# NCAR/SPERR

Hardware: AMD Instinct MI355X
Metric: compress+decompress GB/s/GPU on 256^3 fp32 chunks @ BPP=2.0; bitstream-exact vs ref (higher is better)
Workload: dtype f64; 1 GPU; synthetic 1024^3 fp32 turbulence per GPU, 256^3 chunks, BPP=2.0, step = compress + decompress, volume and container resident in HBM; chunks_per_gpu=64, parallelism=chunks farmed over 1 GPU(s), no collective

## Files before the change

### sperr_amd/csrc/xform.hip

```cpp
#include <type_traits>

#include "xform.h"
#include "speck_dec.h"

namespace sperrhip {


constexpr int kSumStrides = 64, kSumSeg = 64;


template <typename T>
__global__ void __launch_bounds__(kThreads)
k_stride_sums(const T* __restrict__ vol, VolDesc vd, const ChunkGeom* geom, uint32_t cx,
              uint32_t cy, uint32_t cz, uint32_t nstrides, uint32_t ssz, double* strideMean,
              size_t strideMeanStride, CoderState* st, int want_range)
{
  __shared__ double tile[kSumStrides][kSumSeg + 1];
  __shared__ uint32_t sh_differs;
  double vmax = -INFINITY, vnegmax = -INFINITY;
  const uint32_t c = blockIdx.y;
  const uint32_t s0 = blockIdx.x * kSumStrides;
  const ChunkGeom g = geom[c];
  const size_t vx = vd.dims[0], vy = vd.dims[1];
  const T first = vol[((size_t)g.org[2] * vy + g.org[1]) * vx + g.org[0]];
  if (threadIdx.x == 0)
    sh_differs = 0;
  double acc = 0.0;
  bool differs = false;
  (void)cz;
  for (uint32_t seg = 0; seg < ssz; seg += kSumSeg) {
    const uint32_t len = min((uint32_t)kSumSeg, ssz - seg);
    __syncthreads();
    for (uint32_t k = threadIdx.x; k < (uint32_t)(kSumStrides * kSumSeg); k += kThreads) {
      const uint32_t r = k / kSumSeg, j = k % kSumSeg;
      const uint32_t sidx = s0 + r;
      if (sidx < nstrides && j < len) {
        const uint32_t e = sidx * ssz + seg + j;
        const uint32_t x = e % cx, q = e / cx;
        const uint32_t y = q % cy, z = q / cy;
        const T v = vol[((size_t)(g.org[2] + z) * vy + (g.org[1] + y)) * vx + g.org[0] + x];
        differs |= (v != first);
        tile[r][j] = (double)v;
        vmax = fmax(vmax, (double)v);
        vnegmax = fmax(vnegmax, -(double)v);
      }
    }
    __syncthreads();
    if (threadIdx.x < (uint32_t)kSumStrides && s0 + threadIdx.x < nstrides)
      for (uint32_t j = 0; j < len; j++)
        acc += tile[threadIdx.x][j];
  }
  if (differs)
    sh_differs = 1;
  __syncthreads();
  if (threadIdx.x < (uint32_t)kSumStrides && s0 + threadIdx.x < nstrides)
    strideMean[c * strideMeanStride + s0 + threadIdx.x] = acc / (double)ssz;
  if (threadIdx.x == 0 && sh_differs)
    st[c].not_const_flag = 1;
  if (want_range) {
    for (int d = 32; d > 0; d >>= 1) {
      vmax = fmax(vmax, __shfl_xor(vmax, d, 64));
      vnegmax = fmax(vnegmax, __shfl_xor(vnegmax, d, 64));
    }
    if ((threadIdx.x & 63) == 0) {
      atomicMax(reinterpret_cast<unsigned long long*>(&st[c].vmaxKey), order_key(vmax));
      atomicMax(reinterpret_cast<unsigned long long*>(&st[c].vnegmaxKey), order_key(vnegmax));
    }
  }
}

template <typename T>
__global__ void __launch_bounds__(64)
k_stride_sums_rows(const T* __restrict__ vol, VolDesc vd, const ChunkGeom* geom, uint32_t cx,
                   uint32_t cy, uint32_t nstrides, uint32_t ssz, double* strideMean,
                   size_t strideMeanStride, CoderState* st, int want_range)
{
  constexpr int V = 16 / sizeof(T);
  struct alignas(16) Pack { T v[V]; };
  const uint32_t c = blockIdx.y;
  const uint32_t sidx = blockIdx.x * 64 + threadIdx.x;
  const ChunkGeom g = geom[c];
  const size_t vx = vd.dims[0], vy = vd.dims[1];
  const T first = vol[((size_t)g.org[2] * vy + g.org[1]) * vx + g.org[0]];
  double acc = 0.0, vmax = -INFINITY, vnegmax = -INFINITY;
  bool differs = false;
// ... 304 lines not shown
          EV(i) = fma(EV(i), K.inv_eps, -t);
        }
      __syncthreads();
      odd_step(-K.gamma);
      even_step(-K.beta);
      odd_step(-K.alpha);
    }
#undef EV
#undef OD
  }

  auto crop_store = [&](uint32_t l, uint32_t p, VT v) {
    uint32_t xyz[3];
    xyz[axis] = p;
    xyz[ua] = u0 + l;
    xyz[wa] = tw;
    if (crop_has(cg, xyz[0], xyz[1], xyz[2]))
      vol[crop_addr(cg, vd, xyz[0], xyz[1], xyz[2])] = v;
  };
  (void)crop_store;
  const bool wantMax = FORWARD && F.mode == 1 && !is_const;
  double vmax = 0.0;
  if (axis == 0) {
    const uint32_t nseg = (len + 63) / 64;
    for (uint32_t sg = tid / 64; sg < nl * nseg; sg += kThreads / 64) {
      const uint32_t l = sg / nseg, p = (sg % nseg) * 64 + tid % 64;
      if (p >= len)
        continue;
      const uint32_t src = FORWARD ? p : ((p & 1) ? even_len + (p >> 1) : (p >> 1));
      if constexpr (kCrop)
        crop_store(l, p, (VT)(is_const ? mean : sm[src * NLP + l] + mean));
      else if (IO != 0 && !FORWARD)
        vol[vbase + l * vsu + p * vsl] = (VT)(is_const ? mean : sm[src * NLP + l] + mean);
      else {
        const double v = sm[src * NLP + l];
        tile[l * su + p] = v;
        size_t idx;
        if (wantMax && outside_inner(l, p, idx))
          vmax = fmax(vmax, fabs(v));
      }
    }
  }
  else {
    const uint32_t l = tid % NL, k0 = tid / NL, kg = kThreads / NL;
    if (l < nl)
      for (uint32_t p = k0; p < len; p += kg) {
        const uint32_t src = FORWARD ? p : ((p & 1) ? even_len + (p >> 1) : (p >> 1));
        if constexpr (kCrop)
          crop_store(l, p, (VT)(is_const ? mean : sm[src * NLP + l] + mean));
        else if (IO != 0 && !FORWARD)
          vol[vbase + l * vsu + p * vsl] = (VT)(is_const ? mean : sm[src * NLP + l] + mean);
        else {
          const double v = sm[src * NLP + l];
          tile[l * su + p * sl] = v;
          size_t idx;
          if (wantMax && outside_inner(l, p, idx))
            vmax = fmax(vmax, fabs(v));
        }
      }
  }
  if (FORWARD && F.mode == 1) {
    for (int d = 32; d > 0; d >>= 1)
      vmax = fmax(vmax, __shfl_xor(vmax, d, 64));
    if ((tid & 63) == 0 && vmax > 0.0)
      atomicMax(reinterpret_cast<unsigned long long*>(&st[c].maxabs),
                (unsigned long long)__double_as_longlong(vmax));
  }
}

constexpr int kXYHalo = 4;
constexpr int kXYThreads = 512;
constexpr int kStage = 16;
constexpr int kSeg = 8;

__device__ __forceinline__ uint32_t reflect_index(int q, int n)
{
  const int period = 2 * (n - 1);
  q = q < 0 ? -q : q;
  if (q >= period)
    q %= period;
  return (uint32_t)(q < n ? q : period - q);
}

template <bool FORWARD>
__device__ __forceinline__ void lift16(double (&r)[16], const LiftConsts& K)
{
  if (FORWARD) {
#pragma unroll
    for (int k = 1; k <= 13; k += 2)
      r[k] = fma(K.alpha, r[k - 1] + r[k + 1], r[k]);
#pragma unroll
    for (int k = 2; k <= 12; k += 2)
      r[k] = fma(K.beta, r[k - 1] + r[k + 1], r[k]);
#pragma unroll
    for (int k = 3; k <= 11; k += 2)
      r[k] = fma(K.gamma, r[k - 1] + r[k + 1], r[k]);
#pragma unroll
    for (int k = 4; k <= 10; k += 2)
      r[k] = K.eps * fma(K.delta, r[k - 1] + r[k + 1], r[k]);
#pragma unroll
    for (int k = 5; k <= 11; k += 2)
      r[k] = (-K.inv_eps) * r[k];
  }
  else {
#pragma unroll
    for (int k = 1; k <= 15; k += 2)
      r[k] = (-K.eps) * r[k];
#pragma unroll
    for (int k = 2; k <= 14; k += 2) {
      const double t = K.delta * (r[k - 1] + r[k + 1]);
      r[k] = fma(r[k], K.inv_eps, -t);
    }
#pragma unroll
    for (int k = 3; k <= 13; k += 2)
      r[k] = fma(-K.gamma, r[k - 1] + r[k + 1], r[k]);
#pragma unroll
    for (int k = 4; k <= 12; k += 2)
      r[k] = fma(-K.beta, r[k - 1] + r[k + 1], r[k]);
#pragma unroll
    for (int k = 5; k <= 11; k += 2)
      r[k] = fma(-K.alpha, r[k - 1] + r[k + 1], r[k]);
  }
}

template <bool FORWARD, int IO, bool kCrop = false>
__global__ void __launch_bounds__(kXYThreads)
k_lift_xy(double* vals, size_t valsStride, uint32_t cx, uint32_t cy, uint32_t cz, int R,
          LiftConsts K, const CoderState* st, void* volume, VolDesc vd, const GeomOf<kCrop>* geom)
{
  static_assert(IO == 1 || IO == 2, "float or double volume");
  static_assert(!kCrop || !FORWARD, "the crop variant is a last inverse pass");
  using VT = typename std::conditional<IO == 1, float, double>::type;
  const uint32_t c = blockIdx.y;
  const bool is_const = st[c].is_const != 0;
  if (is_const && FORWARD)
    return;
  double* sm = reinterpret_cast<double*>(dyn_smem);
  const uint32_t ntile = (cy + R - 1) / R;
  const uint32_t z = blockIdx.x / ntile, y0 = (blockIdx.x % ntile) * R;
  const uint32_t ylo = y0 >= (uint32_t)kXYHalo ? y0 - kXYHalo : 0u;
  const uint32_t yhi = min(cy, y0 + R + kXYHalo);
  const uint32_t yend = min(cy, y0 + R);
  const uint32_t nrow = yhi - ylo;
  const uint32_t RS = cx + 1;
  const uint32_t xe = cx - cx / 2, ye = cy - cy / 2;
  const GeomOf<kCrop> g = geom[c];
  VT* vol = reinterpret_cast<VT*>(volume);
  const size_t vsy = vd.dims[0], vsz = (size_t)vd.dims[0] * vd.dims[1];
  size_t vbase = 0;
  uint32_t wy0 = y0, wy1 = yend, wx0 = 0, wx1 = cx;
  if constexpr (kCrop) {
    wy0 = max(y0, g.lo[1]);
    wy1 = min(yend, g.hi[1]);
    wx0 = g.lo[0];
    wx1 = g.hi[0];
    if (z - g.lo[2] >= g.hi[2] - g.lo[2] || wy0 >= wy1)
      return;
  }
  else
    vbase = (size_t)(g.org[2] + z) * vsz + (size_t)g.org[1] * vsy + g.org[0];
  auto out_at = [&](uint32_t x, uint32_t y) -> size_t {
    if constexpr (kCrop)
      return crop_addr(g, vd, x, y, z);
    else
      return vbase + (size_t)y * vsy + x;
  };
  double* buf = vals + c * valsStride + (size_t)z * cx * cy;
  const double mean = st[c].mean;
  const uint32_t tid = threadIdx.x;

  if (is_const) {
    if constexpr (kCrop) {
      const uint32_t w = wx1 - wx0;
      for (uint32_t k = tid; k < (wy1 - wy0) * w; k += kXYThreads)
        vol[out_at(wx0 + k % w, wy0 + k / w)] = (VT)mean;
    }
    else
      for (uint32_t k = tid; k < (yend - y0) * cx; k += kXYThreads)
        vol[vbase + (size_t)(y0 + k / cx) * vsy + k % cx] = (VT)mean;
    return;
  }

  const uint32_t lane = tid & 63u, wave = tid >> 6, nwaves = kXYThreads / 64;
  {
    using ST = typename std::conditional<FORWARD, VT, double>::type;
    const uint32_t nxb = (cx + 63) / 64;
    const uint32_t rowsW = nrow > wave ? (nrow - wave + nwaves - 1) / nwaves : 0;
    const uint32_t items = rowsW * nxb;
    uint32_t ri = 0, bi = 0;
    for (uint32_t m0 = 0; m0 < items; m0 += kStage) {
      ST v[kStage];
      uint32_t ri2 = ri, bi2 = bi;
#pragma unroll
      for (int u = 0; u < kStage; u++) {
        const uint32_t j = wave + nwaves * ri2, x = lane + 64 * bi2;
        v[u] = 0;
        if (m0 + u < items && x < cx) {
          const uint32_t y = ylo + j;
          if (FORWARD)
            v[u] = (ST)vol[vbase + (size_t)y * vsy + x];
          else
            v[u] = (ST)buf[(size_t)((y & 1) ? ye + (y >> 1) : (y >> 1)) * cx + ((x & 1) ? xe + (x >> 1) : (x >> 1))];
        }
        if (++bi2 == nxb) {
          bi2 = 0;
          ri2++;
// ... 62 lines not shown
      for (int k = 0; k < 16; k++) {
        const uint32_t yy = min(max(reflect_index(s - 4 + k, (int)cy), ylo), yhi - 1);
        r[k] = col[(size_t)(yy - ylo) * RS];
      }
    }
  };

  if (FORWARD) {
    lift_x(0, nrow);
    for (uint32_t xb = 0; xb < cx; xb += cpr) {
      const uint32_t x = xb + tid % cpr, q = tid / cpr;
      if (x < cx && q < nq) {
        double r[16];
        load_column(x, q, r);
        lift16<true>(r, K);
        const uint32_t dcol = (x & 1) ? xe + (x >> 1) : (x >> 1);
#pragma unroll
        for (int k = 0; k < kSeg; k++) {
          const uint32_t y = y0 + q * kSeg + k;
          if (y < yend)
            buf[(size_t)((y & 1) ? ye + (y >> 1) : (y >> 1)) * cx + dcol] = r[4 + k];
        }
      }
    }
  }
  else {
    for (uint32_t xb = 0; xb < cx; xb += cpr) {
      const uint32_t x = xb + tid % cpr, q = tid / cpr;
      const bool on = x < cx && q < nq;
      double r[16];
      if (on) {
        load_column(x, q, r);
        lift16<false>(r, K);
      }
      __syncthreads();
      if (on) {
#pragma unroll
        for (int k = 0; k < kSeg; k++) {
          const uint32_t y = y0 + q * kSeg + k;
          if (y < yend)
            sm[(size_t)(y - ylo) * RS + x] = r[4 + k];
        }
      }
    }
    __syncthreads();
    lift_x(y0 - ylo, yend - ylo);
    if constexpr (kCrop) {
      for (uint32_t y = wy0 + wave; y < wy1; y += nwaves) {
        VT* dstrow = vol + out_at(wx0, y);
        const double* srow = sm + (size_t)(y - ylo) * RS;
        for (uint32_t x = wx0 + lane; x < wx1; x += 64)
          dstrow[x - wx0] = (VT)(srow[x] + mean);
      }
    }
    else
    for (uint32_t y = y0 + wave; y < yend; y += nwaves) {
      VT* dstrow = vol + vbase + (size_t)y * vsy;
      const double* srow = sm + (size_t)(y - ylo) * RS;
      for (uint32_t x = lane; x < cx; x += 64)
        dstrow[x] = (VT)(srow[x] + mean);
    }
  }
}

#ifndef XYZ_INV_THREADS
#define XYZ_INV_THREADS 1024
#endif
#ifndef XYZ_INV_PREFETCH
#define XYZ_INV_PREFETCH 2
#endif
#ifndef XYZ_FWD_THREADS
#define XYZ_FWD_THREADS 1024
#endif
constexpr int kXYZThreadsF = XYZ_FWD_THREADS, kXYZThreadsI = XYZ_INV_THREADS;
constexpr int kXYZRows = 16;
constexpr int kXYZStaged = kXYZRows + 2 * kXYHalo;
constexpr int kXYZPosF = (4096 + kXYZThreadsF - 1) / kXYZThreadsF;
constexpr int kXYZStageF = (6144 + kXYZThreadsF - 1) / kXYZThreadsF;
constexpr int kXYZPosI = 6144 / kXYZThreadsI;
#ifndef XYZ_INV_GROUP
#define XYZ_INV_GROUP 3
#endif
constexpr int kXYZGroupI = XYZ_INV_GROUP;
constexpr int kXYZBoxSlots = 48;

__host__ __device__ inline uint32_t xyz_row_stride(uint32_t cx)
{
  return ((cx + 7u) & ~7u) + 9u;
}

#define XYZ_LDS_BARRIER() asm volatile("s_waitcnt lgkmcnt(0)\n\ts_barrier" ::: "memory")

__device__ __forceinline__ void xyz_put(double* row, uint32_t x, uint32_t cx, double v)
{
  row[4 + x] = v;
  if (x - 1u < 4u)
    row[4 - x] = v;
  if (cx - 2u - x < 4u)
    row[2 * cx + 2 - x] = v;
}

template <bool FORWARD, int NT>
__device__ __forceinline__ void xyz_lift_x(const double* src, double* dst, uint32_t RS, uint32_t cx, uint32_t jlo,
                                           uint32_t jhi, uint32_t tid, const LiftConsts& K)
{
  const uint32_t nseg = (cx + kSeg - 1) / kSeg;
  const uint32_t ntask = (jhi - jlo) * nseg;
#pragma unroll 1
  for (uint32_t t = tid; t < ntask; t += NT) {
    const uint32_t rows = jhi - jlo, sg = t / rows, rb = jlo + (t - sg * rows);
    const double* row = src + (size_t)rb * RS + sg * kSeg;
    double r[16];
#pragma unroll
    for (int k = 0; k < 16; k++)
      r[k] = row[k];
    lift16<FORWARD>(r, K);
    double* out = dst + (size_t)rb * RS + 4 + sg * kSeg;
#pragma unroll
    for (int k = 0; k < kSeg; k++)
      if (sg * kSeg + k < cx)
        out[k] = r[4 + k];
  }
}

template <bool FORWARD, bool APRON, int NT>
__device__ __forceinline__ void xyz_lift_y(const double* src, double* dst, uint32_t RS, uint32_t cx, uint32_t nt,
                                           uint32_t tid, const LiftConsts& K)
{
  const uint32_t nq = (nt + kSeg - 1) / kSeg;
  const uint32_t ntask = nq * cx;
#pragma unroll 1
  for (uint32_t t = tid; t < ntask; t += NT) {
    const uint32_t q = t / cx, x = t - q * cx;
    const double* top = src + (size_t)(q * kSeg) * RS + 4 + x;
    double r[16];
#pragma unroll
    for (int k = 0; k < 16; k++)
      r[k] = top[(size_t)k * RS];
    lift16<FORWARD>(r, K);
#pragma unroll
    for (int k = 0; k < kSeg; k++) {
      if (q * kSeg + k < nt) {
        double* row = dst + (size_t)(4 + q * kSeg + k) * RS;
        if (APRON)
          xyz_put(row, x, cx, r[4 + k]);
        else
          row[4 + x] = r[4 + k];
      }
    }
  }
}

template <int IO>
__global__ void __launch_bounds__(kXYZThreadsF) __attribute__((amdgpu_waves_per_eu(kXYZThreadsF / 256, kXYZThreadsF / 256)))
k_lift_xyz_fwd(double* vals, size_t valsStride, uint32_t cx, uint32_t cy, uint32_t cz, LiftConsts K,
               CoderState* st, const void* volume, VolDesc vd, const ChunkGeom* geom, int wantMax,
               uint32_t in0, uint32_t in1, uint32_t in2, uint32_t nseg)
{
  static_assert(IO == 1 || IO == 2, "float or double volume");
  using VT = typename std::conditional<IO == 1, float, double>::type;
  const uint32_t c = blockIdx.y;
  if (st[c].is_const != 0)
    return;
  const uint32_t tid = threadIdx.x;
  const uint32_t seg = blockIdx.x % nseg, npairsAll = (cz + 1) / 2;
  const uint32_t mA = seg == 0 ? 0u : (uint32_t)((uint64_t)npairsAll * seg / nseg);
  const uint32_t mB = seg + 1 == nseg ? npairsAll : (uint32_t)((uint64_t)npairsAll * (seg + 1) / nseg);
  const uint32_t zFirst = mA >= 6 ? 2 * (mA - 6) : 0u;
  const uint32_t zEnd = seg + 1 == nseg ? cz : 2 * mB - 1;
  const uint32_t y0 = (blockIdx.x / nseg) * kXYZRows;
  const uint32_t nt = min((uint32_t)kXYZRows, cy - y0);
  const uint32_t RS = xyz_row_stride(cx);
  double* sm = reinterpret_cast<double*>(dyn_smem);
  const uint32_t bufN = (uint32_t)kXYZStaged * RS;
  const uint32_t xe = cx - cx / 2, ye = cy - cy / 2, ze = cz - cz / 2;
  const VT* vol = reinterpret_cast<const VT*>(volume);
  const size_t vsy = vd.dims[0], vsz = (size_t)vd.dims[0] * vd.dims[1];
  const VT* volc = vol + ((size_t)geom[c].org[2] * vsz + (size_t)geom[c].org[1] * vsy + geom[c].org[0]);
  double* buf = vals + c * valsStride;
  const size_t sliceN = (size_t)cx * cy;
  const double mean = st[c].mean;

  const uint32_t nstage = (uint32_t)kXYZStaged * cx;
  uint32_t pk[kXYZStageF];
#pragma unroll
  for (int k = 0; k < kXYZStageF; k++) {
    const uint32_t q = tid + (uint32_t)k * kXYZThreadsF;
    const uint32_t j = q / cx, x = q - j * cx;
    pk[k] = (j << 27) | (reflect_index((int)y0 - kXYHalo + (int)j, (int)cy) << 12) | x;
  }
  const uint32_t npos = nt * cx;
  uint32_t srow[kXYZPosF], ooff[kXYZPosF];
  uint32_t outerMask = 0;
#pragma unroll
  for (int k = 0; k < kXYZPosF; k++) {
    const uint32_t q = tid + (uint32_t)k * kXYZThreadsF;
    const uint32_t row = q / cx, col = q - row * cx, y = y0 + row;
    srow[k] = ((row + kXYHalo) << 16) | col;
    const uint32_t drow = (y & 1) ? ye + (y >> 1) : (y >> 1), dcol = (col & 1) ? xe + (col >> 1) : (col >> 1);
    ooff[k] = drow * cx + dcol;
    if (!(dcol < in0 && drow < in1))
      outerMask |= 1u << k;
  }
  double sxe[kXYZPosF], sxo[kXYZPosF], d1p[kXYZPosF], e1p[kXYZPosF], d2p[kXYZPosF];
#pragma unroll
  for (int k = 0; k < kXYZPosF; k++)
    sxe[k] = sxo[k] = d1p[k] = e1p[k] = d2p[k] = 0.0;
  double vmax = 0.0;
  auto emit = [&](int k, uint32_t zp, double v) {
    buf[(size_t)zp * sliceN + ooff[k]] = v;
    if (wantMax && (((outerMask >> k) & 1u) || zp >= in2))
      vmax = fmax(vmax, fabs(v));
  };

  VT pre[kXYZStageF];
  auto issue = [&](uint32_t z) {
    const VT* src = volc + (size_t)z * vsz;
#pragma unroll
    for (int k = 0; k < kXYZStageF; k++)
      pre[k] = (tid + (uint32_t)k * kXYZThreadsF) < nstage
                   ? src[(size_t)((pk[k] >> 12) & 0x7fffu) * vsy + (pk[k] & 0xfffu)] : (VT)0;
  };
  issue(zFirst);
  for (uint32_t z = zFirst; z < zEnd; z++) {
    uint32_t RSv = RS, tidv = tid;
    asm volatile("" : "+s"(RSv), "+v"(tidv));
#pragma unroll
    for (int k = 0; k < kXYZStageF; k++)
      asm volatile("" : "+v"(pk[k]));
#pragma unroll
    for (int k = 0; k < kXYZPosF; k++)
      asm volatile("" : "+v"(srow[k]), "+v"(ooff[k]));
    double* A = sm + ((z & 1) ? bufN : 0u);
    double* B = sm + ((z & 1) ? 0u : bufN);
#pragma unroll
    for (int k = 0; k < kXYZStageF; k++)
      if ((tid + (uint32_t)k * kXYZThreadsF) < nstage)
        xyz_put(A + (pk[k] >> 27) * RSv, pk[k] & 0xfffu, cx, (double)pre[k] - mean);
    if (z + 1 < zEnd)
      issue(z + 1);
    XYZ_LDS_BARRIER();
    xyz_lift_x<true, kXYZThreadsF>(A, B, RSv, cx, 0, kXYZStaged, tidv, K);
    XYZ_LDS_BARRIER();
    xyz_lift_y<true, false, kXYZThreadsF>(B, A, RSv, cx, nt, tidv, K);
    XYZ_LDS_BARRIER();
    const uint32_t m = z >> 1;
    if (z & 1) {
#pragma unroll
      for (int k = 0; k < kXYZPosF; k++)
        if ((tid + (uint32_t)k * kXYZThreadsF) < npos)
          sxo[k] = A[(srow[k] >> 16) * RSv + 4 + (srow[k] & 0xffffu)];
    }
    else {
#pragma unroll
      for (int k = 0; k < kXYZPosF; k++) {
        if ((tid + (uint32_t)k * kXYZThreadsF) >= npos)
          continue;
        const double v = A[(srow[k] >> 16) * RSv + 4 + (srow[k] & 0xffffu)];
        if (m >= 1) {
          const double d1n = fma(K.alpha, sxe[k] + v, sxo[k]);
          const double e1n = fma(K.beta, (m == 1 ? d1n : d1p[k]) + d1n, sxe[k]);
          if (m >= 2) {
            const double d2n = fma(K.gamma, e1p[k] + e1n, d1p[k]);
            const double e2 = K.eps * fma(K.delta, (m == 2 ? d2n : d2p[k]) + d2n, e1p[k]);
            if (m >= mA) {
              emit(k, m - 2, e2);
              emit(k, ze + m - 2, (-K.inv_eps) * d2n);
            }
            d2p[k] = d2n;
          }
          d1p[k] = d1n;
          e1p[k] = e1n;
        }
        sxe[k] = v;
      }
    }
  }
#pragma unroll
  for (int k = 0; k < kXYZPosF; k++) {
    if ((tid + (uint32_t)k * kXYZThreadsF) >= npos || seg + 1 != nseg)
      continue;
    if ((cz & 1) == 0) {
      const uint32_t M = cz / 2 - 1;
      const double d1L = fma(K.alpha, sxe[k] + sxe[k], sxo[k]);
      const double e1M = fma(K.beta, d1p[k] + d1L, sxe[k]);
      const double d2a = fma(K.gamma, e1p[k] + e1M, d1p[k]);
      const double e2a = K.eps * fma(K.delta, d2p[k] + d2a, e1p[k]);
      const double d2L = fma(K.gamma, e1M + e1M, d1L);
      const double e2L = K.eps * fma(K.delta, d2a + d2L, e1M);
      emit(k, M - 1, e2a);
      emit(k, ze + M - 1, (-K.inv_eps) * d2a);
      emit(k, M, e2L);
      emit(k, ze + M, (-K.inv_eps) * d2L);
    }
    else {
      const uint32_t M = cz / 2;
      const double e1M = fma(K.beta, d1p[k] + d1p[k], sxe[k]);
      const double d2a = fma(K.gamma, e1p[k] + e1M, d1p[k]);
      const double e2a = K.eps * fma(K.delta, d2p[k] + d2a, e1p[k]);
      const double e2L = K.eps * fma(K.delta, d2a + d2a, e1M);
      emit(k, M - 1, e2a);
      emit(k, ze + M - 1, (-K.inv_eps) * d2a);
      emit(k, M, e2L);
    }
  }
  if (wantMax) {
    for (int d = 32; d > 0; d >>= 1)
      vmax = fmax(vmax, __shfl_xor(vmax, d, 64));
    if ((tid & 63) == 0 && vmax > 0.0)
      atomicMax(reinterpret_cast<unsigned long long*>(&st[c].maxabs),
                (unsigned long long)__double_as_longlong(vmax));
  }
}

template <int IO, bool SG, bool kCrop = false>
__global__ void __launch_bounds__(kXYZThreadsI) __attribute__((amdgpu_waves_per_eu(kXYZThreadsI / 256, kXYZThreadsI / 256)))
k_lift_xyz_inv(const double* vals, size_t valsStride, uint32_t cx, uint32_t cy, uint32_t cz, LiftConsts K,
               const CoderState* st, void* volume, VolDesc vd, const GeomOf<kCrop>* geom, LiftFuse F, uint32_t nseg)
{
  static_assert(IO == 1 || IO == 2, "float or double volume");
  using VT = typename std::conditional<IO == 1, float, double>::type;
  const uint32_t c = blockIdx.y;
  const uint32_t tid = threadIdx.x;
  const uint32_t seg = blockIdx.x % nseg, npairsAll = cz / 2;
  const uint32_t mA = seg == 0 ? 0u : (uint32_t)((uint64_t)npairsAll * seg / nseg);
  const uint32_t mB = seg + 1 == nseg ? npairsAll : (uint32_t)((uint64_t)npairsAll * (seg + 1) / nseg);
  const uint32_t mFirst = mA >= 6 ? mA - 6 : 0u;
  const uint32_t y0 = (blockIdx.x / nseg) * kXYZRows;
  const uint32_t nt = min((uint32_t)kXYZRows, cy - y0);
  const uint32_t RS = xyz_row_stride(cx);
  double* sm = reinterpret_cast<double*>(dyn_smem);
  const uint32_t bufN = (uint32_t)kXYZStaged * RS;
  const uint32_t xe = cx - cx / 2, ye = cy - cy / 2, ze = cz - cz / 2;
  VT* vol = reinterpret_cast<VT*>(volume);
  const size_t vsy = vd.dims[0], vsz = (size_t)vd.dims[0] * vd.dims[1];
  VT* volc = vol;
  CropGeom cg{};
  uint32_t wy0 = 0, wy1 = 0;
  if constexpr (kCrop) {
    cg = geom[c];
    wy0 = max(y0, cg.lo[1]) - y0;
    wy1 = min(y0 + nt, cg.hi[1]);
    if (y0 + wy0 >= wy1)
      return;
    wy1 -= y0;
  }
  else
    volc = vol + ((size_t)geom[c].org[2] * vsz + (size_t)geom[c].org[1] * vsy + geom[c].org[0]);
  auto crop_row = [&](uint32_t z, uint32_t r) -> VT* { return vol + crop_addr(cg, vd, cg.lo[0], y0 + r, z); };
  (void)crop_row;
  const double* buf = vals + c * valsStride;
  const size_t sliceN = (size_t)cx * cy;
  const uint32_t bufx = F.bufx ? F.bufx : cx;
  const size_t bufSlice = (size_t)bufx * (F.bufy ? F.bufy : cy);
  const double mean = st[c].mean;
  const uint32_t lane = tid & 63u, wave = tid >> 6, nwaves = kXYZThreadsI / 64;

  if (st[c].is_const != 0) {
    if constexpr (kCrop) {
      const uint32_t w = cg.hi[0] - cg.lo[0], nr = wy1 - wy0;
      for (uint32_t z = cg.lo[2] + seg; z < cg.hi[2]; z += nseg)
        for (uint32_t k = tid; k < nr * w; k += kXYZThreadsI)
          crop_row(z, wy0 + k / w)[k % w] = (VT)mean;
    }
    else
    for (uint32_t z = seg; z < cz; z += nseg)
      for (uint32_t k = tid; k < nt * cx; k += kXYZThreadsI)
        volc[(size_t)z * vsz + (size_t)(y0 + k / cx) * vsy + k % cx] = (VT)mean;
    return;
  }

  const uint32_t npos = (uint32_t)kXYZStaged * cx;
  uint32_t pk[kXYZPosI];
  uint32_t innerMask = 0;
#pragma unroll
  for (int k = 0; k < kXYZPosI; k++) {
    const uint32_t q = tid + (uint32_t)k * kXYZThreadsI;
    const uint32_t j = q / cx, x = q - j * cx, y = reflect_index((int)y0 - kXYHalo + (int)j, (int)cy);
    const uint32_t drow = (y & 1) ? ye + (y >> 1) : (y >> 1), dcol = (x & 1) ? xe + (x >> 1) : (x >> 1);
    pk[k] = (j << 27) | (y << 12) | x;
    if (dcol < F.inner[0] && drow < F.inner[1])
      innerMask |= 1u << k;
  }
  const bool dequant = F.mode == 2 && !st[c].wide;
  const double fq = dequant ? st[c].q : 0.0;
  const uint32_t* coef = F.coef + c * F.coefStride;
  const uint64_t* sign = F.sign + c * F.signStride;
  const bool haveMasks = dequant && F.sigNew != nullptr && F.dst != nullptr;
  const uint64_t* mNew = haveMasks ? F.sigNew + c * F.maskStride : sign;
  const uint64_t* mOld = haveMasks ? F.sigOld + c * F.maskStride : sign;
  const uint32_t lastPl = haveMasks ? (uint32_t)F.dst[c].lastPlane : 0u;
  const uint32_t initNew = haveMasks ? (1u << lastPl) + (1u << lastPl) - (1u << lastPl) / 2 - 1 : 0u;
  const uint32_t initOld = (haveMasks && lastPl < 31) ? (2u << lastPl) + (2u << lastPl) - (2u << lastPl) / 2 - 1 : 0u;
  const int scheme = (SG && dequant && F.dst) ? coef_scheme(F.dst[c]) : 0;
  const bool two = scheme == 2;
  auto sg_value = [&](uint32_t sv) -> double {
    double d = fq * (double)coef_scheme_mag(sv, two);
    return __hiloint2double(__double2hiint(d) ^ (int)(sv & 0x80000000u), __double2loint(d));
  };
  auto fetch = [&](int k, uint32_t zp) -> double {
    const uint32_t y = (pk[k] >> 12) & 0x7fffu, x = pk[k] & 0xfffu;
    const uint32_t drow = (y & 1) ? ye + (y >> 1) : (y >> 1), dcol = (x & 1) ? xe + (x >> 1) : (x >> 1);
    const size_t idx = (size_t)zp * sliceN + drow * cx + dcol;
    const bool inBox = ((innerMask >> k) & 1u) && zp < F.inner[2];
    if (!dequant && !inBox && F.bufx)
      return 0.0;
    if (dequant && !inBox) {
      if (SG && scheme)
        return sg_value(coef[idx]);
      uint32_t v = coef[idx];
      const uint32_t sh = (uint32_t)(idx & 63);
      const uint64_t sgw = sign[idx >> 6], mnw = mNew[idx >> 6], mow = mOld[idx >> 6];
      const uint32_t fill = ((mnw >> sh) & 1ull) ? initNew : (((mow >> sh) & 1ull) ? initOld : 0u);
      v = v ? v : fill;
      return fq * (double)v * (((sgw >> sh) & 1ull) ? 1.0 : -1.0);
    }
    return buf[(size_t)zp * bufSlice + drow * bufx + dcol];
  };
  uint32_t flip = 0;
  auto stage = [&](int k, double v) {
    uint32_t p = pk[k];
    asm volatile("" : "+v"(p));
    (sm + (flip ? bufN : 0u))[(p >> 27) * RS + 4 + (p & 0xfffu)] = v;
  };
  auto stage_all = [&](const double (&v)[kXYZPosI]) {
#pragma unroll
    for (int k = 0; k < kXYZPosI; k++)
      if ((tid + (uint32_t)k * kXYZThreadsI) < npos)
        stage(k, v[k]);
  };
  auto store_rows = [&](uint32_t z, uint32_t which) {
    const double* X = sm + (which ? bufN : 0u);
    if constexpr (kCrop) {
      if (z - cg.lo[2] >= cg.hi[2] - cg.lo[2])
        return;
      for (uint32_t r = wy0 + wave; r < wy1; r += nwaves) {
        VT* dstrow = crop_row(z, r);
        const double* srow = X + (size_t)(kXYHalo + r) * RS + 4;
        for (uint32_t x = cg.lo[0] + lane; x < cg.hi[0]; x += 64)
          dstrow[x - cg.lo[0]] = (VT)(F.noMean ? srow[x] : srow[x] + mean);
      }
      return;
    }
    for (uint32_t r = wave; r < nt; r += nwaves) {
      VT* dstrow = volc + (size_t)z * vsz + (size_t)(y0 + r) * vsy;
      const double* srow = X + (size_t)(kXYHalo + r) * RS + 4;
      if (F.noMean) {
        for (uint32_t x = lane; x < cx; x += 64)
          dstrow[x] = (VT)srow[x];
      }
      else
        for (uint32_t x = lane; x < cx; x += 64)
          dstrow[x] = (VT)(srow[x] + mean);
    }
  };
  auto finish_slice = [&](uint32_t z) {
    uint32_t RSv = RS, tidv = tid;
    asm volatile("" : "+s"(RSv), "+v"(tidv));
    const uint32_t which = flip;
    double* X = sm + (flip ? bufN : 0u);
    double* Y = sm + (flip ? 0u : bufN);
    flip ^= 1u;
    XYZ_LDS_BARRIER();
    xyz_lift_y<false, true, kXYZThreadsI>(X, Y, RSv, cx, nt, tidv, K);
    XYZ_LDS_BARRIER();
    xyz_lift_x<false, kXYZThreadsI>(Y, X, RSv, cx, kXYHalo, kXYHalo + nt, tidv, K);
    XYZ_LDS_BARRIER();
    store_rows(z, which);
  };

  double o1p[kXYZPosI], e1p[kXYZPosI], o2p[kXYZPosI], e2p[kXYZPosI];
#pragma unroll
  for (int k = 0; k < kXYZPosI; k++)
    o1p[k] = e1p[k] = o2p[k] = e2p[k] = 0.0;
  const uint32_t npairs = cz / 2;
  auto zstep = [&](int k, uint32_t m, bool mine, bool active, double E, double O) {
    const double o1 = (-K.eps) * O;
    const double t = K.delta * ((m == 0 ? o1 : o1p[k]) + o1);
    const double e1 = fma(E, K.inv_eps, -t);
    if (m >= 1) {
      const double o2 = fma(-K.gamma, e1p[k] + e1, o1p[k]);
      const double e2 = fma(-K.beta, (m == 1 ? o2 : o2p[k]) + o2, e1p[k]);
      if (m >= 2 && mine && active)
        stage(k, fma(-K.alpha, e2p[k] + e2, o2p[k]));
      o2p[k] = o2;
      e2p[k] = e2;
    }
    o1p[k] = o1;
    e1p[k] = e1;
  };
#if XYZ_INV_PREFETCH == 2
  uint32_t* myPre = reinterpret_cast<uint32_t*>(sm + 2 * (size_t)bufN) + (size_t)wave * (kXYZPosI * 2 * 64);
  const uint32_t* sign32 = reinterpret_cast<const uint32_t*>(sign);
  const uint32_t* mNew32 = reinterpret_cast<const uint32_t*>(mNew);
  const uint32_t* mOld32 = reinterpret_cast<const uint32_t*>(mOld);
  uint32_t activeMask = 0;
#pragma unroll
  for (int k = 0; k < kXYZPosI; k++)
    if ((tid + (uint32_t)k * kXYZThreadsI) < npos)
      activeMask |= 1u << k;
    else
      pk[k] = pk[0];
  uint32_t boxAny = 0;
#pragma unroll
  for (int k = 0; k < kXYZPosI; k++)
    boxAny |= __ballot((innerMask >> k) & 1u) != 0ull ? 1u << k : 0u;
  boxAny = (uint32_t)__builtin_amdgcn_readfirstlane((int)boxAny);
  auto pos_off = [&](int k, uint32_t& drow, uint32_t& dcol) {
    const uint32_t y = (pk[k] >> 12) & 0x7fffu, x = pk[k] & 0xfffu;
    drow = (y & 1) ? ye + (y >> 1) : (y >> 1);
    dcol = (x & 1) ? xe + (x >> 1) : (x >> 1);
  };
  const bool fastLoads = dequant && F.inner[2] <= ze && (!SG || scheme != 0);
  uint32_t boxLds = 0, boxSlot0 = 0;
  uint32_t* boxRows = reinterpret_cast<uint32_t*>(sm + 2 * (size_t)bufN) + (size_t)nwaves * (kXYZPosI * 2 * 64);
  if (SG && fastLoads) {
    uint32_t reg = 0;
#pragma unroll
    for (int k = 0; k < kXYZPosI; k++) {
      const uint64_t inb = __ballot((innerMask >> k) & 1u), act = __ballot((activeMask >> k) & 1u);
      if (inb == 0x5555555555555555ull && act == ~0ull && (cx & 63u) == 0)
        reg |= 1u << k;
    }
    reg = (uint32_t)__builtin_amdgcn_readfirstlane((int)reg);
    uint32_t* cnt = reinterpret_cast<uint32_t*>(sm);
    if (lane == 0)
      cnt[wave] = (uint32_t)__popc(reg);
    XYZ_LDS_BARRIER();
    uint32_t before = 0, total = 0;
    for (uint32_t w = 0; w < nwaves; w++) {
      const uint32_t v = cnt[w];
      before += w < wave ? v : 0u;
      total += v;
    }
    XYZ_LDS_BARRIER();
    if (total <= (uint32_t)kXYZBoxSlots && reg == (1u << kXYZPosI) - 1u) {
      boxLds = reg;
      boxSlot0 = before;
    }
  }
  uint32_t* myBox = boxRows + (size_t)boxSlot0 * 64;
  auto pre_issue = [&](uint32_t m) {
#pragma unroll
    for (int k = 0; k < kXYZPosI; k++) {
      uint32_t drow, dcol;
      pos_off(k, drow, dcol);
      const uint32_t off = drow * cx + dcol;
      __builtin_amdgcn_global_load_lds(coef + ((size_t)m * sliceN + off), myPre + (k * 2) * 64, 4, 0, 0);
      __builtin_amdgcn_global_load_lds(coef + ((size_t)(ze + m) * sliceN + off), myPre + (k * 2 + 1) * 64, 4, 0, 0);
    }
    if (SG && boxLds != 0 && m < F.inner[2]) {
#pragma unroll
      for (int k = 0; k < kXYZPosI; k++) {
        uint32_t drow, dcol;
        pos_off(k, drow, dcol);
        const uint32_t x0h = ((pk[k] & 0xfffu) - lane) >> 1;
        const uint32_t* src = reinterpret_cast<const uint32_t*>(buf + ((size_t)m * bufSlice + (size_t)drow * bufx + x0h)) + lane;
        __builtin_amdgcn_global_load_lds(src, myBox + k * 64, 4, 0, 0);
      }
    }
  };
  if (fastLoads && mFirst < mB)
    pre_issue(mFirst);
#endif
  for (uint32_t m = mFirst; m < mB; m++) {
    const bool mine = m >= mA;
#pragma unroll
    for (int k = 0; k < kXYZPosI; k++)
      asm volatile("" : "+v"(pk[k]));
#if XYZ_INV_PREFETCH == 2
    if (SG && fastLoads) {
      asm volatile("s_waitcnt vmcnt(0)" ::: "memory");
      const bool boxWave = boxAny != 0 && m < F.inner[2];
      if (boxWave && boxLds != 0) {
#pragma unroll
        for (int k = 0; k < kXYZPosI; k++) {
          const double lo = sg_value(myPre[(k * 2) * 64 + lane]);
          const double hi = sg_value(myPre[(k * 2 + 1) * 64 + lane]);
          const double bxv = reinterpret_cast<const double*>(myBox + k * 64)[lane >> 1];
          zstep(k, m, mine, true, (lane & 1u) ? lo : bxv, hi);
        }
      }
      else {
#pragma unroll
      for (int g = 0; g < kXYZPosI; g += kXYZGroupI) {
        __builtin_amdgcn_sched_barrier(0);
        double bx[kXYZGroupI];
        uint32_t boxm = 0;
        if (boxWave) {
#pragma unroll
          for (int kk = 0; kk < kXYZGroupI; kk++) {
            const int k = g + kk;
            if (k >= kXYZPosI)
              continue;
            uint32_t drow, dcol;
            pos_off(k, drow, dcol);
            const bool inBox = ((innerMask >> k) & 1u) != 0;
            boxm |= inBox ? 1u << kk : 0u;
            bx[kk] = buf[inBox ? (size_t)m * bufSlice + drow * bufx + dcol : (size_t)0];
          }
        }
#pragma unroll
        for (int kk = 0; kk < kXYZGroupI; kk++) {
          const int k = g + kk;
          if (k >= kXYZPosI)
            continue;
          const double lo = sg_value(myPre[(k * 2) * 64 + lane]);
          const double hi = sg_value(myPre[(k * 2 + 1) * 64 + lane]);
          zstep(k, m, mine, ((activeMask >> k) & 1u) != 0, ((boxm >> kk) & 1u) ? bx[kk] : lo, hi);
        }
      }
      }
      __builtin_amdgcn_sched_barrier(0);
      if (m + 1 < mB)
        pre_issue(m + 1);
      __builtin_amdgcn_sched_barrier(0);
    }
    else if (!SG && fastLoads) {
      asm volatile("s_waitcnt vmcnt(0)" ::: "memory");
#pragma unroll
      for (int g = 0; g < kXYZPosI; g += kXYZGroupI) {
        __builtin_amdgcn_sched_barrier(0);
        constexpr int NV = 2 * kXYZGroupI;
        uint32_t sgw[NV], mnw[NV], mow[NV], cv[NV], shv[NV], boxm = 0;
        double bx[kXYZGroupI];
#pragma unroll
        for (int j = 0; j < NV; j++) {
          const int k = g + j / 2;
          if (k >= kXYZPosI)
            continue;
          const uint32_t zp = (j & 1) ? ze + m : m;
          uint32_t drow, dcol;
          pos_off(k, drow, dcol);
          const size_t idx = (size_t)zp * sliceN + drow * cx + dcol;
          sgw[j] = sign32[idx >> 5];
          mnw[j] = mNew32[idx >> 5];
          mow[j] = mOld32[idx >> 5];
          if ((j & 1) == 0) {
            const bool inBox = ((innerMask >> k) & 1u) && zp < F.inner[2];
            boxm |= inBox ? 1u << j : 0u;
            bx[j / 2] = buf[inBox ? (size_t)zp * bufSlice + drow * bufx + dcol : (size_t)0];
          }
          cv[j] = myPre[(k * 2 + (j & 1)) * 64 + lane];
          shv[j] = (uint32_t)idx & 31u;
        }
        double val[NV];
#pragma unroll
        for (int j = 0; j < NV; j++) {
          if (g + j / 2 >= kXYZPosI)
            continue;
          const uint32_t fill = ((mnw[j] >> shv[j]) & 1u) ? initNew : (((mow[j] >> shv[j]) & 1u) ? initOld : 0u);
          const uint32_t v = cv[j] ? cv[j] : fill;
          const double dq = fq * (double)v * (((sgw[j] >> shv[j]) & 1u) ? 1.0 : -1.0);
          val[j] = ((j & 1) == 0 && ((boxm >> j) & 1u)) ? bx[j / 2] : dq;
        }
#pragma unroll
        for (int kk = 0; kk < kXYZGroupI; kk++)
          if (g + kk < kXYZPosI)
            zstep(g + kk, m, mine, ((activeMask >> (g + kk)) & 1u) != 0, val[2 * kk], val[2 * kk + 1]);
      }
      __builtin_amdgcn_sched_barrier(0);
      if (m + 1 < mB)
        pre_issue(m + 1);
      __builtin_amdgcn_sched_barrier(0);
    }
    else
// ... 692 lines not shown
```

Baseline: 66.84 GB/s.

## Shrink lifting windows per task and fuse inverse x-lift with volume store

Generalizes the 16-wide lifting window into a templated window of NOUT+8 taps, with configurable outputs per task for the forward and inverse x and y passes. This trades more halo recomputation for more parallel tasks and lower register pressure. The inverse x-lift now writes straight to the output volume with vector stores, dropping one LDS round trip, a barrier and the separate store pass. It also reorders the box prefetch ahead of the coefficient loads and makes wave indices scalar. Compile-time OFF masks add ablation switches that are disabled by default.

```diff
diff --git a/sperr_amd/csrc/lift_window.h b/sperr_amd/csrc/lift_window.h
--- /dev/null
+++ b/sperr_amd/csrc/lift_window.h
@@ -0,0 +1,93 @@
+#ifndef SPERR_AMD_LIFT_WINDOW_H
+#define SPERR_AMD_LIFT_WINDOW_H
+
+#include "xform.h"
+
+namespace sperrhip {
+
+template <bool FORWARD>
+__host__ __device__ __forceinline__ void lift16(double (&r)[16], const LiftConsts& K)
+{
+  if (FORWARD) {
+#pragma unroll
+    for (int k = 1; k <= 13; k += 2)
+      r[k] = fma(K.alpha, r[k - 1] + r[k + 1], r[k]);
+#pragma unroll
+    for (int k = 2; k <= 12; k += 2)
+      r[k] = fma(K.beta, r[k - 1] + r[k + 1], r[k]);
+#pragma unroll
+    for (int k = 3; k <= 11; k += 2)
+      r[k] = fma(K.gamma, r[k - 1] + r[k + 1], r[k]);
+#pragma unroll
+    for (int k = 4; k <= 10; k += 2)
+      r[k] = K.eps * fma(K.delta, r[k - 1] + r[k + 1], r[k]);
+#pragma unroll
+    for (int k = 5; k <= 11; k += 2)
+      r[k] = (-K.inv_eps) * r[k];
+  }
+  else {
+#pragma unroll
+    for (int k = 1; k <= 15; k += 2)
+      r[k] = (-K.eps) * r[k];
+#pragma unroll
+    for (int k = 2; k <= 14; k += 2) {
+      const double t = K.delta * (r[k - 1] + r[k + 1]);
+      r[k] = fma(r[k], K.inv_eps, -t);
+    }
+#pragma unroll
+    for (int k = 3; k <= 13; k += 2)
+      r[k] = fma(-K.gamma, r[k - 1] + r[k + 1], r[k]);
+#pragma unroll
+    for (int k = 4; k <= 12; k += 2)
+      r[k] = fma(-K.beta, r[k - 1] + r[k + 1], r[k]);
+#pragma unroll
+    for (int k = 5; k <= 11; k += 2)
+      r[k] = fma(-K.alpha, r[k - 1] + r[k + 1], r[k]);
+  }
+}
+
+template <bool FORWARD, int W>
+__host__ __device__ __forceinline__ void lift_window(double (&r)[W], const LiftConsts& K)
+{
+  static_assert(W >= 10 && W <= 16 && (W & 1) == 0, "an even number of outputs");
+  if (FORWARD) {
+#pragma unroll
+    for (int k = 1; k <= W - 3; k += 2)
+      r[k] = fma(K.alpha, r[k - 1] + r[k + 1], r[k]);
+#pragma unroll
+    for (int k = 2; k <= W - 4; k += 2)
+      r[k] = fma(K.beta, r[k - 1] + r[k + 1], r[k]);
+#pragma unroll
+    for (int k = 3; k <= W - 5; k += 2)
+      r[k] = fma(K.gamma, r[k - 1] + r[k + 1], r[k]);
+#pragma unroll
+    for (int k = 4; k <= W - 6; k += 2)
+      r[k] = K.eps * fma(K.delta, r[k - 1] + r[k + 1], r[k]);
+#pragma unroll
+    for (int k = 5; k <= W - 5; k += 2)
+      r[k] = (-K.inv_eps) * r[k];
+  }
+  else {
+#pragma unroll
+    for (int k = 1; k <= W - 1; k += 2)
+      r[k] = (-K.eps) * r[k];
+#pragma unroll
+    for (int k = 2; k <= W - 2; k += 2) {
+      const double t = K.delta * (r[k - 1] + r[k + 1]);
+      r[k] = fma(r[k], K.inv_eps, -t);
+    }
+#pragma unroll
+    for (int k = 3; k <= W - 3; k += 2)
+      r[k] = fma(-K.gamma, r[k - 1] + r[k + 1], r[k]);
+#pragma unroll
+    for (int k = 4; k <= W - 4; k += 2)
+      r[k] = fma(-K.beta, r[k - 1] + r[k + 1], r[k]);
+#pragma unroll
+    for (int k = 5; k <= W - 5; k += 2)
+      r[k] = fma(-K.alpha, r[k - 1] + r[k + 1], r[k]);
+  }
+}
+
+}
+
+#endif
diff --git a/sperr_amd/csrc/xform.hip b/sperr_amd/csrc/xform.hip
--- a/sperr_amd/csrc/xform.hip
+++ b/sperr_amd/csrc/xform.hip
@@ -1,6 +1,7 @@
 #include <type_traits>
 
 #include "xform.h"
+#include "lift_window.h"
 #include "speck_dec.h"
 
 namespace sperrhip {
@@ -471,46 +472,6 @@
   return (uint32_t)(q < n ? q : period - q);
 }
 
-template <bool FORWARD>
-__device__ __forceinline__ void lift16(double (&r)[16], const LiftConsts& K)
-{
-  if (FORWARD) {
-#pragma unroll
-    for (int k = 1; k <= 13; k += 2)
-      r[k] = fma(K.alpha, r[k - 1] + r[k + 1], r[k]);
-#pragma unroll
-    for (int k = 2; k <= 12; k += 2)
-      r[k] = fma(K.beta, r[k - 1] + r[k + 1], r[k]);
-#pragma unroll
-    for (int k = 3; k <= 11; k += 2)
-      r[k] = fma(K.gamma, r[k - 1] + r[k + 1], r[k]);
-#pragma unroll
-    for (int k = 4; k <= 10; k += 2)
-      r[k] = K.eps * fma(K.delta, r[k - 1] + r[k + 1], r[k]);
-#pragma unroll
-    for (int k = 5; k <= 11; k += 2)
-      r[k] = (-K.inv_eps) * r[k];
-  }
-  else {
-#pragma unroll
-    for (int k = 1; k <= 15; k += 2)
-      r[k] = (-K.eps) * r[k];
-#pragma unroll
-    for (int k = 2; k <= 14; k += 2) {
-      const double t = K.delta * (r[k - 1] + r[k + 1]);
-      r[k] = fma(r[k], K.inv_eps, -t);
-    }
-#pragma unroll
-    for (int k = 3; k <= 13; k += 2)
-      r[k] = fma(-K.gamma, r[k - 1] + r[k + 1], r[k]);
-#pragma unroll
-    for (int k = 4; k <= 12; k += 2)
-      r[k] = fma(-K.beta, r[k - 1] + r[k + 1], r[k]);
-#pragma unroll
-    for (int k = 5; k <= 11; k += 2)
-      r[k] = fma(-K.alpha, r[k - 1] + r[k + 1], r[k]);
-  }
-}
 
 template <bool FORWARD, int IO, bool kCrop = false>
 __global__ void __launch_bounds__(kXYThreads)
@@ -739,6 +700,35 @@
 #define XYZ_INV_GROUP 3
 #endif
 constexpr int kXYZGroupI = XYZ_INV_GROUP;
+#ifndef XYZ_FWD_YOUT
+#define XYZ_FWD_YOUT 4
+#endif
+#ifndef XYZ_FWD_XOUT
+#define XYZ_FWD_XOUT 8
+#endif
+#ifndef XYZ_INV_YOUT
+#define XYZ_INV_YOUT 4
+#endif
+#ifndef XYZ_INV_XOUT
+#define XYZ_INV_XOUT 4
+#endif
+#ifndef XYZ_INV_XSTORE
+#define XYZ_INV_XSTORE 1
+#endif
+#ifndef XYZ_FWD_OFF
+#define XYZ_FWD_OFF 0
+#endif
+#ifndef XYZ_INV_OFF
+#define XYZ_INV_OFF 0
+#endif
+template <int MASK>
+__device__ __forceinline__ bool xyz_off(int bit, uint32_t nseg)
+{
+  return (MASK & bit) != 0 && nseg != ~0u;
+}
+constexpr int kXYZOutFY = XYZ_FWD_YOUT, kXYZOutFX = XYZ_FWD_XOUT, kXYZOutIY = XYZ_INV_YOUT, kXYZOutIX = XYZ_INV_XOUT;
+constexpr bool xyz_out_ok(int n) { return n == 2 || n == 4 || n == 8; }
+static_assert(xyz_out_ok(kXYZOutFY) && xyz_out_ok(kXYZOutFX) && xyz_out_ok(kXYZOutIY) && xyz_out_ok(kXYZOutIX), "2, 4 or 8 outputs a task");
 constexpr int kXYZBoxSlots = 48;
 
 __host__ __device__ inline uint32_t xyz_row_stride(uint32_t cx)
@@ -757,48 +747,88 @@
     row[2 * cx + 2 - x] = v;
 }
 
-template <bool FORWARD, int NT>
+template <bool FORWARD, int NT, int NOUT>
 __device__ __forceinline__ void xyz_lift_x(const double* src, double* dst, uint32_t RS, uint32_t cx, uint32_t jlo,
                                            uint32_t jhi, uint32_t tid, const LiftConsts& K)
 {
-  const uint32_t nseg = (cx + kSeg - 1) / kSeg;
+  const uint32_t nseg = (cx + NOUT - 1) / NOUT;
   const uint32_t ntask = (jhi - jlo) * nseg;
 #pragma unroll 1
   for (uint32_t t = tid; t < ntask; t += NT) {
     const uint32_t rows = jhi - jlo, sg = t / rows, rb = jlo + (t - sg * rows);
-    const double* row = src + (size_t)rb * RS + sg * kSeg;
-    double r[16];
-#pragma unroll
-    for (int k = 0; k < 16; k++)
+    const double* row = src + (size_t)rb * RS + sg * NOUT;
+    double r[NOUT + 8];
+#pragma unroll
+    for (int k = 0; k < NOUT + 8; k++)
       r[k] = row[k];
-    lift16<FORWARD>(r, K);
-    double* out = dst + (size_t)rb * RS + 4 + sg * kSeg;
-#pragma unroll
-    for (int k = 0; k < kSeg; k++)
-      if (sg * kSeg + k < cx)
+    lift_window<FORWARD, NOUT + 8>(r, K);
+    double* out = dst + (size_t)rb * RS + 4 + sg * NOUT;
+#pragma unroll
+    for (int k = 0; k < NOUT; k++)
+      if (sg * NOUT + k < cx)
         out[k] = r[4 + k];
   }
 }
 
-template <bool FORWARD, bool APRON, int NT>
+template <int NT, int NOUT, typename VT>
+__device__ __forceinline__ void xyz_lift_x_store(const double* src, VT* vrows, size_t vsy, uint32_t RS, uint32_t cx, uint32_t jlo,
+                                                 uint32_t jhi, uint32_t tid, const LiftConsts& K, double mean, bool noMean,
+                                                 bool doStore)
+{
+  const uint32_t nseg = (cx + NOUT - 1) / NOUT;
+  const uint32_t ntask = (jhi - jlo) * nseg;
+#pragma unroll 1
+  for (uint32_t t = tid; t < ntask; t += NT) {
+    const uint32_t rows = jhi - jlo, sg = t / rows, rb = t - sg * rows;
+    const double* row = src + (size_t)(jlo + rb) * RS + sg * NOUT;
+    double r[NOUT + 8];
+#pragma unroll
+    for (int k = 0; k < NOUT + 8; k++)
+      r[k] = row[k];
+    lift_window<false, NOUT + 8>(r, K);
+    VT* out = vrows + (size_t)rb * vsy + sg * NOUT;
+    VT v[NOUT];
+#pragma unroll
+    for (int k = 0; k < NOUT; k++)
+      v[k] = (VT)(noMean ? r[4 + k] : r[4 + k] + mean);
+    if (!doStore)
+      continue;
+    if (sg * NOUT + NOUT <= cx) {
+      typedef VT Seg __attribute__((ext_vector_type(NOUT), aligned(sizeof(VT))));
+      Seg s;
+#pragma unroll
+      for (int k = 0; k < NOUT; k++)
+        s[k] = v[k];
+      *reinterpret_cast<Seg*>(out) = s;
+    }
+    else {
+#pragma unroll
+      for (int k = 0; k < NOUT; k++)
+        if (sg * NOUT + k < cx)
+          out[k] = v[k];
+    }
+  }
+}
+
+template <bool FORWARD, bool APRON, int NT, int NOUT>
 __device__ __forceinline__ void xyz_lift_y(const double* src, double* dst, uint32_t RS, uint32_t cx, uint32_t nt,
                                            uint32_t tid, const LiftConsts& K)
 {
-  const uint32_t nq = (nt + kSeg - 1) / kSeg;
+  const uint32_t nq = (nt + NOUT - 1) / NOUT;
   const uint32_t ntask = nq * cx;
 #pragma unroll 1
   for (uint32_t t = tid; t < ntask; t += NT) {
     const uint32_t q = t / cx, x = t - q * cx;
-    const double* top = src + (size_t)(q * kSeg) * RS + 4 + x;
-    double r[16];
-#pragma unroll
-    for (int k = 0; k < 16; k++)
+    const double* top = src + (size_t)(q * NOUT) * RS + 4 + x;
+    double r[NOUT + 8];
+#pragma unroll
+    for (int k = 0; k < NOUT + 8; k++)
       r[k] = top[(size_t)k * RS];
-    lift16<FORWARD>(r, K);
-#pragma unroll
-    for (int k = 0; k < kSeg; k++) {
-      if (q * kSeg + k < nt) {
-        double* row = dst + (size_t)(4 + q * kSeg + k) * RS;
+    lift_window<FORWARD, NOUT + 8>(r, K);
+#pragma unroll
+    for (int k = 0; k < NOUT; k++) {
+      if (q * NOUT + k < nt) {
+        double* row = dst + (size_t)(4 + q * NOUT + k) * RS;
         if (APRON)
           xyz_put(row, x, cx, r[4 + k]);
         else
@@ -865,7 +895,8 @@
     sxe[k] = sxo[k] = d1p[k] = e1p[k] = d2p[k] = 0.0;
   double vmax = 0.0;
   auto emit = [&](int k, uint32_t zp, double v) {
-    buf[(size_t)zp * sliceN + ooff[k]] = v;
+    if (!xyz_off<XYZ_FWD_OFF>(4, nseg))
+      buf[(size_t)zp * sliceN + ooff[k]] = v;
     if (wantMax && (((outerMask >> k) & 1u) || zp >= in2))
       vmax = fmax(vmax, fabs(v));
   };
@@ -874,9 +905,15 @@
   auto issue = [&](uint32_t z) {
     const VT* src = volc + (size_t)z * vsz;
 #pragma unroll
-    for (int k = 0; k < kXYZStageF; k++)
-      pre[k] = (tid + (uint32_t)k * kXYZThreadsF) < nstage
-                   ? src[(size_t)((pk[k] >> 12) & 0x7fffu) * vsy + (pk[k] & 0xfffu)] : (VT)0;
+    for (int k = 0; k < kXYZStageF; k++) {
+      if (xyz_off<XYZ_FWD_OFF>(1, nseg)) {
+        pre[k] = (VT)(((pk[k] + z * 40503u) * 2654435761u) >> 20);
+      }
+      else {
+        pre[k] = (tid + (uint32_t)k * kXYZThreadsF) < nstage
+                     ? src[(size_t)((pk[k] >> 12) & 0x7fffu) * vsy + (pk[k] & 0xfffu)] : (VT)0;
+      }
+    }
   };
   issue(zFirst);
   for (uint32_t z = zFirst; z < zEnd; z++) {
@@ -897,11 +934,15 @@
     if (z + 1 < zEnd)
       issue(z + 1);
     XYZ_LDS_BARRIER();
-    xyz_lift_x<true, kXYZThreadsF>(A, B, RSv, cx, 0, kXYZStaged, tidv, K);
+    if (!xyz_off<XYZ_FWD_OFF>(2, nseg))
+      xyz_lift_x<true, kXYZThreadsF, kXYZOutFX>(A, B, RSv, cx, 0, kXYZStaged, tidv, K);
     XYZ_LDS_BARRIER();
-    xyz_lift_y<true, false, kXYZThreadsF>(B, A, RSv, cx, nt, tidv, K);
+    if (!xyz_off<XYZ_FWD_OFF>(2, nseg))
+      xyz_lift_y<true, false, kXYZThreadsF, kXYZOutFY>(B, A, RSv, cx, nt, tidv, K);
     XYZ_LDS_BARRIER();
     const uint32_t m = z >> 1;
+    if (xyz_off<XYZ_FWD_OFF>(8, nseg))
+      continue;
     if (z & 1) {
 #pragma unroll
       for (int k = 0; k < kXYZPosF; k++)
@@ -1011,7 +1052,8 @@
   const uint32_t bufx = F.bufx ? F.bufx : cx;
   const size_t bufSlice = (size_t)bufx * (F.bufy ? F.bufy : cy);
   const double mean = st[c].mean;
-  const uint32_t lane = tid & 63u, wave = tid >> 6, nwaves = kXYZThreadsI / 64;
+  const uint32_t lane = tid & 63u, nwaves = kXYZThreadsI / 64;
+  const uint32_t wave = (uint32_t)__builtin_amdgcn_readfirstlane((int)(tid >> 6));
 
   if (st[c].is_const != 0) {
     if constexpr (kCrop) {
@@ -1088,42 +1130,59 @@
   };
   auto store_rows = [&](uint32_t z, uint32_t which) {
     const double* X = sm + (which ? bufN : 0u);
+    uint32_t lanev = lane;
+    asm volatile("" : "+v"(lanev));
     if constexpr (kCrop) {
       if (z - cg.lo[2] >= cg.hi[2] - cg.lo[2])
         return;
       for (uint32_t r = wy0 + wave; r < wy1; r += nwaves) {
         VT* dstrow = crop_row(z, r);
         const double* srow = X + (size_t)(kXYHalo + r) * RS + 4;
-        for (uint32_t x = cg.lo[0] + lane; x < cg.hi[0]; x += 64)
+        for (uint32_t x = cg.lo[0] + lanev; x < cg.hi[0]; x += 64)
           dstrow[x - cg.lo[0]] = (VT)(F.noMean ? srow[x] : srow[x] + mean);
       }
       return;
     }
+    if (xyz_off<XYZ_INV_OFF>(4, nseg))
+      return;
     for (uint32_t r = wave; r < nt; r += nwaves) {
       VT* dstrow = volc + (size_t)z * vsz + (size_t)(y0 + r) * vsy;
       const double* srow = X + (size_t)(kXYHalo + r) * RS + 4;
       if (F.noMean) {
-        for (uint32_t x = lane; x < cx; x += 64)
+        for (uint32_t x = lanev; x < cx; x += 64)
           dstrow[x] = (VT)srow[x];
       }
       else
-        for (uint32_t x = lane; x < cx; x += 64)
+        for (uint32_t x = lanev; x < cx; x += 64)
           dstrow[x] = (VT)(srow[x] + mean);
     }
   };
+  constexpr bool kDirect = !kCrop && XYZ_INV_XSTORE != 0;
   auto finish_slice = [&](uint32_t z) {
     uint32_t RSv = RS, tidv = tid;
     asm volatile("" : "+s"(RSv), "+v"(tidv));
     const uint32_t which = flip;
     double* X = sm + (flip ? bufN : 0u);
     double* Y = sm + (flip ? 0u : bufN);
-    flip ^= 1u;
+    if constexpr (!kDirect)
+      flip ^= 1u;
     XYZ_LDS_BARRIER();
-    xyz_lift_y<false, true, kXYZThreadsI>(X, Y, RSv, cx, nt, tidv, K);
+    if (!xyz_off<XYZ_INV_OFF>(2, nseg))
+      xyz_lift_y<false, true, kXYZThreadsI, kXYZOutIY>(X, Y, RSv, cx, nt, tidv, K);
     XYZ_LDS_BARRIER();
-    xyz_lift_x<false, kXYZThreadsI>(Y, X, RSv, cx, kXYHalo, kXYHalo + nt, tidv, K);
-    XYZ_LDS_BARRIER();
-    store_rows(z, which);
+    if constexpr (kDirect) {
+      if (!xyz_off<XYZ_INV_OFF>(2, nseg))
+        xyz_lift_x_store<kXYZThreadsI, kXYZOutIX>(Y, volc + (size_t)z * vsz + (size_t)y0 * vsy, vsy, RSv, cx, kXYHalo, kXYHalo + nt,
+                                                   tidv, K, mean, F.noMean != 0, !xyz_off<XYZ_INV_OFF>(4, nseg));
+      else
+        store_rows(z, which ^ 1u);
+    }
+    else {
+      if (!xyz_off<XYZ_INV_OFF>(2, nseg))
+        xyz_lift_x<false, kXYZThreadsI, kXYZOutIX>(Y, X, RSv, cx, kXYHalo, kXYHalo + nt, tidv, K);
+      XYZ_LDS_BARRIER();
+      store_rows(z, which);
+    }
   };
 
   double o1p[kXYZPosI], e1p[kXYZPosI], o2p[kXYZPosI], e2p[kXYZPosI];
@@ -1193,11 +1252,23 @@
     XYZ_LDS_BARRIER();
     if (total <= (uint32_t)kXYZBoxSlots && reg == (1u << kXYZPosI) - 1u) {
       boxLds = reg;
-      boxSlot0 = before;
+      boxSlot0 = (uint32_t)__builtin_amdgcn_readfirstlane((int)before);
     }
   }
   uint32_t* myBox = boxRows + (size_t)boxSlot0 * 64;
   auto pre_issue = [&](uint32_t m) {
+    if (xyz_off<XYZ_INV_OFF>(1, nseg))
+      return;
+    if (SG && boxLds != 0 && m < F.inner[2]) {
+#pragma unroll
+      for (int k = 0; k < kXYZPosI; k++) {
+        uint32_t drow, dcol;
+        pos_off(k, drow, dcol);
+        const uint32_t x0h = ((pk[k] & 0xfffu) - lane) >> 1;
+        const uint32_t* src = reinterpret_cast<const uint32_t*>(buf + ((size_t)m * bufSlice + (size_t)drow * bufx + x0h)) + lane;
+        __builtin_amdgcn_global_load_lds(src, myBox + k * 64, 4, 0, 0);
+      }
+    }
 #pragma unroll
     for (int k = 0; k < kXYZPosI; k++) {
       uint32_t drow, dcol;
@@ -1206,16 +1277,6 @@
       __builtin_amdgcn_global_load_lds(coef + ((size_t)m * sliceN + off), myPre + (k * 2) * 64, 4, 0, 0);
       __builtin_amdgcn_global_load_lds(coef + ((size_t)(ze + m) * sliceN + off), myPre + (k * 2 + 1) * 64, 4, 0, 0);
     }
-    if (SG && boxLds != 0 && m < F.inner[2]) {
-#pragma unroll
-      for (int k = 0; k < kXYZPosI; k++) {
-        uint32_t drow, dcol;
-        pos_off(k, drow, dcol);
-        const uint32_t x0h = ((pk[k] & 0xfffu) - lane) >> 1;
-        const uint32_t* src = reinterpret_cast<const uint32_t*>(buf + ((size_t)m * bufSlice + (size_t)drow * bufx + x0h)) + lane;
-        __builtin_amdgcn_global_load_lds(src, myBox + k * 64, 4, 0, 0);
-      }
-    }
   };
   if (fastLoads && mFirst < mB)
     pre_issue(mFirst);
@@ -1229,7 +1290,8 @@
     if (SG && fastLoads) {
       asm volatile("s_waitcnt vmcnt(0)" ::: "memory");
       const bool boxWave = boxAny != 0 && m < F.inner[2];
-      if (boxWave && boxLds != 0) {
+      const bool zOn = !xyz_off<XYZ_INV_OFF>(8, nseg);
+      if (zOn && boxWave && boxLds != 0) {
 #pragma unroll
         for (int k = 0; k < kXYZPosI; k++) {
           const double lo = sg_value(myPre[(k * 2) * 64 + lane]);
@@ -1238,7 +1300,7 @@
           zstep(k, m, mine, true, (lane & 1u) ? lo : bxv, hi);
         }
       }
-      else {
+      else if (zOn) {
 #pragma unroll
       for (int g = 0; g < kXYZPosI; g += kXYZGroupI) {
         __builtin_amdgcn_sched_barrier(0);
```

Result: faster. 67.65 GB/s (median of 6 runs) (+1.2%).
